# microsoft/StemGNN

Hardware: AMD Instinct MI355X
Metric: forecast-steps/sec (train) (higher is better)
Workload: dtype f32

## Files before the change

stemgnn_amd/csrc/gru.hip:

```cpp
#include <hip/hip_runtime.h>

#include "../../include/stemgnn_hip.h"
#include "gemm2.h"
#include "wgrad.h"
#include "dq_reduce.h"
#include "gemm_core.h"
#include "gru_wide.h"
#include "sg_host.h"

__device__ __forceinline__ float gru_sigmoid(float v) { return 1.f / (1.f + expf(-v)); }
__device__ __forceinline__ int gru_uniform(int v) { return __builtin_amdgcn_readfirstlane(v); }

struct GruGiOp {
  const float *x, *w_ih, *b_ih;
  float* gi;
  int B, S, Hd, W;
  unsigned *za, *zb;
  unsigned na, nb;
  __device__ bool setup(int, int& M, int& N, int& K0, int& K1) const {
    M = S * B; N = 3 * Hd; K0 = 0; K1 = W;
    if (na + nb) {
      const unsigned nwg = gridDim.x * gridDim.y, id = blockIdx.y * gridDim.x + blockIdx.x;
      const unsigned per = (na + nb + nwg - 1) / nwg, hi = min(na + nb, (id + 1) * per);
      for (unsigned i = id * per + threadIdx.x; i < hi; i += blockDim.x) {
// ... 201 lines not shown
    }
    __syncthreads();
    for (int item = wave; item < nwork; item += 16) {
      const int ub = item % nub, jq = item / nub;
      const int unit = ub * 64 + lane;
      const int uc = unit < Hd ? unit : Hd - 1;
      const int j0 = jq * jchunk, j1 = min(H3, j0 + jchunk);
      float a0 = 0.f;
      const float* wp = w_hh + (size_t)j0 * Hd + uc;
#pragma unroll 8
      for (int j = j0; j < j1; ++j) {
        a0 = fmaf(wp[0], dgh[j], a0);
        wp += Hd;
      }
      if (unit < Hd) part[jq * Hd + unit] = a0;
    }
    __syncthreads();
  }
}

typedef unsigned long long gru_u64;
__device__ __forceinline__ void gru_lds_barrier() {
#ifdef GRU_PLAIN_BARRIER
  __syncthreads();
#else
  asm volatile("s_waitcnt lgkmcnt(0)\n\ts_barrier" ::: "memory");
#endif
}
__device__ __forceinline__ void gru_publish(gru_u64* g, unsigned tag, float v) {
  __hip_atomic_store(g, ((gru_u64)tag << 32) | (gru_u64)__float_as_uint(v), __ATOMIC_RELAXED, __HIP_MEMORY_SCOPE_AGENT);
}
__device__ __forceinline__ float gru_consume(const gru_u64* g, unsigned tag, int* status) {
  gru_u64 x = __hip_atomic_load(g, __ATOMIC_RELAXED, __HIP_MEMORY_SCOPE_AGENT);
  unsigned spins = 0;
  while ((unsigned)(x >> 32) != tag) {
#ifndef GRU_NO_SLEEP
    __builtin_amdgcn_s_sleep(1);
#endif
    x = __hip_atomic_load(g, __ATOMIC_RELAXED, __HIP_MEMORY_SCOPE_AGENT);
    if (++spins > (1u << 22)) { atomicExch(status, 1); break; }
  }
  return __uint_as_float((unsigned)x);
}

__device__ __forceinline__ void gru_publish_x(gru_u64* g, unsigned tag, float v, bool same_xcd) {
  const gru_u64 x = ((gru_u64)tag << 32) | (gru_u64)__float_as_uint(v);
#if defined(GRU_PUB_PUSH) && GRU_PUB_PUSH == 3
  if (same_xcd) asm volatile("global_store_dwordx2 %0, %1, off sc0" : : "v"(g), "v"(x) : "memory");
#else
  if (same_xcd) asm volatile("global_store_dwordx2 %0, %1, off" : : "v"(g), "v"(x) : "memory");
#endif
  else __hip_atomic_store(g, x, __ATOMIC_RELAXED, __HIP_MEMORY_SCOPE_AGENT);
}
__device__ __forceinline__ bool gru_same_xcd(gru_u64* xid, int p, int P, int allow, int* status, int* s_flag, int tid) {
  if (tid == 0) {
    const unsigned xcc = __builtin_amdgcn_s_getreg(20 | (0 << 6) | (3 << 11)) & 0xfu;
    gru_publish(xid + p, 1u, (float)(xcc + 1));
    int same = allow;
    for (int q = 0; q < P; ++q) same &= gru_consume(xid + q, 1u, status) == (float)(xcc + 1);
    *s_flag = same;
  }
  __syncthreads();
  return *s_flag != 0;
}

struct GruCluster {
  int P, U, ncb, ksf, kcf, ksb, kcb;
};
__host__ __device__ inline GruCluster gru_cluster_geom(int Hd, int P) {
  GruCluster c;
  c.P = P;
  c.U = (Hd + P - 1) / P;
  c.ncb = (c.U + 63) / 64;
  c.ksf = 16 / (3 * c.ncb);
  c.kcf = c.ksf > 0 ? (Hd + c.ksf - 1) / c.ksf : 1 << 30;
  c.ksb = 16 / c.ncb;
  c.kcb = c.ksb > 0 ? (3 * Hd + c.ksb - 1) / c.ksb : 1 << 30;
  return c;
}
__device__ __forceinline__ void gru_cluster_ids(int B, int P, int& b, int& p) {
  const int id = blockIdx.x;
  const int bl = id & 7, r = id >> 3;
  p = r % P;
  b = (r / P) * 8 + bl;
  (void)B;
}

template <int KC, bool RS = true>
__global__ __launch_bounds__(1024) void gru_fwd_cluster_kernel(const float* __restrict__ gi, const float* __restrict__ w_hh,
                                                               const float* __restrict__ b_hh, int B, int S, int Hd, int P,
                                                               gru_u64* __restrict__ xbuf, int* __restrict__ status,
                                                               float* __restrict__ h_all, float* __restrict__ reserve) {
  extern __shared__ __attribute__((aligned(16))) float smem[];
  int b, p;
  gru_cluster_ids(B, P, b, p);
  if (b >= B) return;
  const GruCluster c = gru_cluster_geom(Hd, P);
  const int tid = threadIdx.x, lane = tid & 63, wave = tid >> 6;
  const int u0 = p * c.U;
  const int un = max(0, min(Hd, u0 + c.U) - u0);
  const int H3 = 3 * Hd;
  float* hs = smem;
  float* part = smem + Hd + KC;
  for (int i = tid; i < Hd + KC; i += 1024) hs[i] = 0.f;
  const int ncol = 3 * c.ncb;
  const bool has = wave < ncol * c.ksf;
  const int cb = has ? wave % ncol : 0, kq = has ? wave / ncol : 0;
  const int g = cb / c.ncb, ul = (cb % c.ncb) * 64 + lane;
  const int k0 = kq * c.kcf, kn = has ? max(0, min(Hd, k0 + c.kcf) - k0) : 0;
  float wr[KC];
  {
    const bool lane_ok = has && ul < un;
    const float* wrow = w_hh + ((size_t)g * Hd + (lane_ok ? u0 + ul : 0)) * Hd + (kn > 0 ? k0 : 0);
#pragma unroll
    for (int kk = 0; kk < KC; ++kk) {
      const float v = wrow[kk < kn ? kk : 0];
      wr[kk] = (lane_ok && kk < kn) ? v : 0.f;
    }
  }
  const int iu = tid < un ? tid : 0;
  const int gu = u0 + iu;
  const float bh0 = b_hh[gu], bh1 = b_hh[Hd + gu], bh2 = b_hh[2 * Hd + gu];
  __syncthreads();

  for (int s = 0; s < S; ++s) {
    const size_t row = (size_t)s * B + b;
    const float* gip = gi + row * H3;
    const float gp0 = gip[gu], gp1 = gip[Hd + gu], gp2 = gip[2 * Hd + gu];
    if (s > 0 && P > 1) {
      const gru_u64* xb = xbuf + ((size_t)(s & 1) * B + b) * Hd;
      for (int i = tid; i < Hd; i += 1024)
        if (i < u0 || i >= u0 + un) hs[i] = gru_consume(xb + i, (unsigned)s, status);
    }
    __syncthreads();
    if (has) {
      float a0 = 0.f, a1 = 0.f;
      const float* hk = hs + k0;
#pragma unroll
      for (int kk = 0; kk < KC; kk += 2) {
        if ((kk & 15) == 0) __builtin_amdgcn_sched_barrier(0);
        a0 = fmaf(wr[kk], hk[kk], a0);
        a1 = fmaf(wr[kk + 1], hk[kk + 1], a1);
      }
      if (ul < un) part[(kq * 3 + g) * c.U + ul] = a0 + a1;
    }
    __syncthreads();
    if (tid < un) {
      float g0 = bh0, g1 = bh1, g2 = bh2;
      for (int q = 0; q < c.ksf; ++q) {
        g0 += part[(q * 3 + 0) * c.U + iu];
        g1 += part[(q * 3 + 1) * c.U + iu];
        g2 += part[(q * 3 + 2) * c.U + iu];
      }
      const float r = gru_sigmoid(gp0 + g0);
      const float z = gru_sigmoid(gp1 + g1);
      const float n = tanhf(gp2 + r * g2);
      const float hn = (1.f - z) * n + z * hs[gu];
      if constexpr (RS) {
        float* rs = reserve + row * 4 * Hd;
        rs[gu] = r; rs[Hd + gu] = z; rs[2 * Hd + gu] = n; rs[3 * Hd + gu] = g2;
      }
      h_all[row * Hd + gu] = hn;
      hs[gu] = hn;
      if (P > 1 && s + 1 < S) gru_publish(xbuf + ((size_t)((s + 1) & 1) * B + b) * Hd + gu, (unsigned)(s + 1), hn);
    }
  }
}

template <int KC>
__global__ __launch_bounds__(1024) void gru_bwd_cluster_kernel(const float* __restrict__ dout, const float* __restrict__ w_hh,
                                                               const float* __restrict__ h_all, const float* __restrict__ reserve,
                                                               int B, int S, int Hd, int P, gru_u64* __restrict__ xbuf,
                                                               int* __restrict__ status, float* __restrict__ dgi,
                                                               float* __restrict__ dghn) {
  extern __shared__ __attribute__((aligned(16))) float smem[];
  int b, p;
  gru_cluster_ids(B, P, b, p);
  if (b >= B) return;
  const GruCluster c = gru_cluster_geom(Hd, P);
  const int tid = threadIdx.x, lane = tid & 63, wave = tid >> 6;
  const int u0 = p * c.U;
  const int un = max(0, min(Hd, u0 + c.U) - u0);
  const int H3 = 3 * Hd;
  float* dgh = smem;
  float* dhz = smem + H3 + KC;
  float* part = dhz + c.U;
  for (int i = tid; i < H3 + KC; i += 1024) dgh[i] = 0.f;
  for (int i = tid; i < c.U; i += 1024) dhz[i] = 0.f;
  for (int i = tid; i < c.ksb * c.U; i += 1024) part[i] = 0.f;
  const bool has = wave < c.ncb * c.ksb;
  const int cb = has ? wave % c.ncb : 0, jq = has ? wave / c.ncb : 0;
  const int ul = cb * 64 + lane;
  const int j0 = jq * c.kcb, jn = has ? max(0, min(H3, j0 + c.kcb) - j0) : 0;
  float wr[KC];
  {
    const bool lane_ok = has && ul < un;
    const float* wcol = w_hh + (size_t)(jn > 0 ? j0 : 0) * Hd + (lane_ok ? u0 + ul : 0);
#pragma unroll
    for (int jj = 0; jj < KC; ++jj) {
      const float v = wcol[(size_t)(jj < jn ? jj : 0) * Hd];
      wr[jj] = (lane_ok && jj < jn) ? v : 0.f;
    }
  }
  const int iu = tid < un ? tid : 0;
  const int gu = u0 + iu;
  __syncthreads();

  for (int s = S - 1; s >= 0; --s) {
    const size_t row = (size_t)s * B + b;
    const unsigned tag = (unsigned)(S - s);
    gru_u64* xb = xbuf + ((size_t)(tag & 1) * B + b) * H3;
    if (tid < un) {
      float dh = dout[row * Hd + gu] + dhz[iu];
      for (int q = 0; q < c.ksb; ++q) dh += part[q * c.U + iu];
      const float* rs = reserve + row * 4 * Hd;
      const float r = rs[gu], z = rs[Hd + gu], n = rs[2 * Hd + gu], ghn = rs[3 * Hd + gu];
      const float hp = h_all[(s > 0 ? row - B : row) * Hd + gu];
      const float hprev = s > 0 ? hp : 0.f;
      const float dn = dh * (1.f - z) * (1.f - n * n);
      const float dz = dh * (hprev - n) * z * (1.f - z);
      const float dr = dn * ghn * r * (1.f - r);
      const float dnr = dn * r;
      dgh[gu] = dr; dgh[Hd + gu] = dz; dgh[2 * Hd + gu] = dnr;
      dhz[iu] = dh * z;
      float* go = dgi + row * H3;
      go[gu] = dr; go[Hd + gu] = dz; go[2 * Hd + gu] = dn;
      dghn[row * Hd + gu] = dnr;
      if (P > 1 && s > 0) {
        gru_publish(xb + gu, tag, dr);
        gru_publish(xb + Hd + gu, tag, dz);
        gru_publish(xb + 2 * Hd + gu, tag, dnr);
      }
    }
    if (s == 0) break;
    if (P > 1) {
      for (int j = tid; j < H3; j += 1024) {
        const int k = j % Hd;
        if (k < u0 || k >= u0 + un) dgh[j] = gru_consume(xb + j, tag, status);
      }
    }
    __syncthreads();
    if (has) {
      float a0 = 0.f, a1 = 0.f;
      const float* gk = dgh + j0;
#pragma unroll
      for (int jj = 0; jj < KC; jj += 2) {
        if ((jj & 15) == 0) __builtin_amdgcn_sched_barrier(0);
        a0 = fmaf(wr[jj], gk[jj], a0);
        a1 = fmaf(wr[jj + 1], gk[jj + 1], a1);
      }
      if (ul < un) part[jq * c.U + ul] = a0 + a1;
    }
    __syncthreads();
  }
}

__device__ __forceinline__ float gru_bcast(float v, int src_lane) {
  return __builtin_bit_cast(float, __builtin_amdgcn_readlane(__builtin_bit_cast(int, v), src_lane));
}
typedef float gru_f2 __attribute__((ext_vector_type(2)));
#ifndef GRU_NR_FWD
#define GRU_NR_FWD 8
#endif
#ifndef GRU_NR_BWD
#define GRU_NR_BWD 16
#endif
#ifndef GRU_NR4
#define GRU_NR4 16
#endif
#define GRU_NR2(P, OW) (((OW) == 1 && (P) <= 4) ? GRU_NR_BWD : 64)
#define GRU_NR3(KU) ((KU) <= 58 ? GRU_NR_FWD : 32)
template <int KU, int NR>
struct GruBcast {
  static constexpr int NRK = NR < KU ? (NR & ~3) : ((KU + 3) & ~3);
  static constexpr int NL = NRK < KU ? (KU - NRK + 3) / 4 : 0;
  float4 v[NL > 0 ? NL : 1];
  float hv;
  __device__ __forceinline__ GruBcast(float hv_, float* lrow, int lane) : hv(hv_) {
    if constexpr (NL > 0) {
      lrow[lane] = hv_;
      asm volatile("" ::: "memory");
#pragma unroll
      for (int i = 0; i < NL; ++i) v[i] = *reinterpret_cast<const float4*>(lrow + NRK + 4 * i);
      __builtin_amdgcn_sched_barrier(0);
    }
  }
  __device__ __forceinline__ gru_f2 pair(int kk) const {
    if (kk < NRK) return gru_f2{gru_bcast(hv, kk), gru_bcast(hv, kk + 1)};
    const float4 t = v[NL > 0 ? (kk - NRK) >> 2 : 0];
    return ((kk - NRK) & 2) ? gru_f2{t.z, t.w} : gru_f2{t.x, t.y};
  }
};
template <int KU, int NR>
__device__ __forceinline__ float gru_matvec(const gru_f2 (&wr)[32], float hv, float* lrow, int lane) {
  const GruBcast<KU, NR> bc(hv, lrow, lane);
  gru_f2 a0 = {0.f, 0.f}, a1 = {0.f, 0.f};
#pragma unroll
  for (int kk = 0; kk + 3 < KU; kk += 4) {
    a0 = __builtin_elementwise_fma(wr[kk >> 1], bc.pair(kk), a0);
    a1 = __builtin_elementwise_fma(wr[(kk >> 1) + 1], bc.pair(kk + 2), a1);
  }
  if constexpr ((KU & 3) != 0) a0 = __builtin_elementwise_fma(wr[(KU - 2) >> 1], bc.pair(KU - 2), a0);
  return (a0.x + a1.x) + (a0.y + a1.y);
}
__device__ __forceinline__ float gru_poll_lane(const gru_u64* g, unsigned tag, bool active, int* status) {
  float v = 0.f;
  if (active) v = gru_consume(g, tag, status);
  return v;
}

#ifdef GRU_PROF
#define GRU_T(var) const long long var = (long long)__builtin_readcyclecounter()
#define GRU_ACC(acc, t1, t0) acc += (t1) - (t0)
#else
#define GRU_T(var)
#define GRU_ACC(acc, t1, t0)
#endif
template <int KU, int NR>
__device__ __forceinline__ void gru_matvec3(const gru_f2 (&w0)[32], const gru_f2 (&w1)[32], const gru_f2 (&w2)[32],
                                            float hv, float* lrow, int lane, float& o0, float& o1, float& o2) {
  const GruBcast<KU, NR> bc(hv, lrow, lane);
  gru_f2 a0 = {0.f, 0.f}, b0 = {0.f, 0.f}, a1 = {0.f, 0.f}, b1 = {0.f, 0.f}, a2 = {0.f, 0.f}, b2 = {0.f, 0.f};
#pragma unroll
  for (int kk = 0; kk + 3 < KU; kk += 4) {
    const gru_f2 h0 = bc.pair(kk), h1 = bc.pair(kk + 2);
    a0 = __builtin_elementwise_fma(w0[kk >> 1], h0, a0);
    a1 = __builtin_elementwise_fma(w1[kk >> 1], h0, a1);
    a2 = __builtin_elementwise_fma(w2[kk >> 1], h0, a2);
    b0 = __builtin_elementwise_fma(w0[(kk >> 1) + 1], h1, b0);
    b1 = __builtin_elementwise_fma(w1[(kk >> 1) + 1], h1, b1);
    b2 = __builtin_elementwise_fma(w2[(kk >> 1) + 1], h1, b2);
  }
  if constexpr ((KU & 3) != 0) {
    const gru_f2 h0 = bc.pair(KU - 2);
    a0 = __builtin_elementwise_fma(w0[(KU - 2) >> 1], h0, a0);
    a1 = __builtin_elementwise_fma(w1[(KU - 2) >> 1], h0, a1);
    a2 = __builtin_elementwise_fma(w2[(KU - 2) >> 1], h0, a2);
  }
  o0 = (a0.x + b0.x) + (a0.y + b0.y);
  o1 = (a1.x + b1.x) + (a1.y + b1.y);
  o2 = (a2.x + b2.x) + (a2.y + b2.y);
}
constexpr int GRU_PACK_KMAX = 40;
template <int KU, int NR>
__device__ __forceinline__ void gru_matvec2(const gru_f2 (&w0)[GRU_PACK_KMAX / 2], const gru_f2 (&w1)[GRU_PACK_KMAX / 2],
                                            float hv, float* lrow, int lane, float& o0, float& o1) {
  static_assert(KU <= GRU_PACK_KMAX && (KU & 1) == 0, "packed mat-vec: slices of at most 40 units");
  const GruBcast<KU, NR> bc(hv, lrow, lane);
  gru_f2 a0 = {0.f, 0.f}, b0 = {0.f, 0.f}, a1 = {0.f, 0.f}, b1 = {0.f, 0.f};
#pragma unroll
  for (int kk = 0; kk + 3 < KU; kk += 4) {
    const gru_f2 h0 = bc.pair(kk), h1 = bc.pair(kk + 2);
    a0 = __builtin_elementwise_fma(w0[kk >> 1], h0, a0);
    a1 = __builtin_elementwise_fma(w1[kk >> 1], h0, a1);
    b0 = __builtin_elementwise_fma(w0[(kk >> 1) + 1], h1, b0);
    b1 = __builtin_elementwise_fma(w1[(kk >> 1) + 1], h1, b1);
  }
  if constexpr ((KU & 3) != 0) {
    const gru_f2 h0 = bc.pair(KU - 2);
    a0 = __builtin_elementwise_fma(w0[(KU - 2) >> 1], h0, a0);
    a1 = __builtin_elementwise_fma(w1[(KU - 2) >> 1], h0, a1);
  }
  o0 = (a0.x + b0.x) + (a0.y + b0.y);
  o1 = (a1.x + b1.x) + (a1.y + b1.y);
}
template <int P, int KU, int OW>
__global__ __launch_bounds__(3 * (P / OW) * 64) void gru_bwd_cluster2_kernel(const float* __restrict__ dout, const float* __restrict__ w_hh,
                                                                      const float* __restrict__ h_all,
                                                                      const float* __restrict__ reserve, int B, int S, int Hd,
                                                                      gru_u64* __restrict__ xbuf, int* __restrict__ status,
                                                                      float* __restrict__ dgi, float* __restrict__ dghn,
                                                                      int s_hi, int s_lo, float* __restrict__ carry,
                                                                      int s_mark, unsigned* __restrict__ progress,
                                                                      gru_u64* __restrict__ xid, int allow_fast) {
  static_assert(P % OW == 0, "owners per wave");
  constexpr int NTH = 3 * (P / OW) * 64;
  __shared__ float part[2][3 * P][64];
  __shared__ __attribute__((aligned(16))) float lrow[3 * P][64];
  __shared__ int s_fast;
  int b, p;
  gru_cluster_ids(B, P, b, p);
  if (b >= B) return;
  const bool fast = P > 1 && gru_same_xcd(xid + (size_t)b * P, p, P, allow_fast, status, &s_fast, threadIdx.x);
  const int U = (Hd + P - 1) / P;
  const int tid = threadIdx.x, lane = tid & 63;
  const int wave = gru_uniform(tid >> 6);
  const int g = wave / (P / OW), q0 = (wave - g * (P / OW)) * OW;
  const int u0 = p * U, un = max(0, min(Hd, u0 + U) - u0);
  const int H3 = 3 * Hd;
  gru_f2 wr[OW][32];
  int k0[OW], kn[OW];
#pragma unroll
  for (int o = 0; o < OW; ++o) {
    k0[o] = ((q0 + o + p) % P) * U;
    kn[o] = max(0, min(Hd, k0[o] + U) - k0[o]);
    const bool lane_ok = lane < un;
    const float* wcol = w_hh + ((size_t)g * Hd + (kn[o] > 0 ? k0[o] : 0)) * Hd + (lane_ok ? u0 + lane : 0);
#pragma unroll
    for (int kk = 0; kk < KU; ++kk) {
      const float v = wcol[(size_t)(kk < kn[o] ? kk : 0) * Hd];
      wr[o][kk >> 1][kk & 1] = (lane_ok && kk < kn[o]) ? v : 0.f;
    }
  }
  const int gu = u0 + (tid < un ? tid : 0);
  float dhz = s_hi < S - 1 ? carry[(size_t)b * Hd + gu] : 0.f;
  for (int i = tid; i < 2 * 3 * P * 64; i += NTH) (&part[0][0][0])[i] = 0.f;
  size_t prow = (size_t)s_hi * B + b;
  float p_do = dout[prow * Hd + gu];
  float p_r = reserve[prow * 4 * Hd + gu], p_z = reserve[prow * 4 * Hd + Hd + gu];
  float p_n = reserve[prow * 4 * Hd + 2 * Hd + gu], p_g = reserve[prow * 4 * Hd + 3 * Hd + gu];
  float p_h = h_all[(s_hi > 0 ? prow - B : prow) * Hd + gu];
  __syncthreads();

#ifdef GRU_PROF
  long long c_poll = 0, c_mv = 0, c_bar = 0, c_gate = 0;
#endif
  for (int s = s_hi; s >= s_lo; --s) {
    const size_t row = (size_t)s * B + b;
    const unsigned tag = (unsigned)(S - s);
    gru_u64* xb = xbuf + ((size_t)(tag & 1) * B + b) * H3;
    float own_dr = 0.f;
    GRU_T(t0);
    if (tid < un) {
      float dh = p_do + dhz;
#pragma unroll
      for (int w = 0; w < 3 * P; ++w) dh += part[(tag + 1) & 1][w][tid];
      const float r = p_r, z = p_z, n = p_n, ghn = p_g;
      const float hprev = s > 0 ? p_h : 0.f;
      const float dn = dh * (1.f - z) * (1.f - n * n);
      const float dz = dh * (hprev - n) * z * (1.f - z);
      const float dr = dn * ghn * r * (1.f - r);
      const float dnr = dn * r;
      own_dr = dr;
      dhz = dh * z;
      if (s > 0) {
        gru_publish_x(xb + gu, tag, dr, fast);
        gru_publish_x(xb + Hd + gu, tag, dz, fast);
        gru_publish_x(xb + 2 * Hd + gu, tag, dnr, fast);
        const size_t rn = row - B;
        p_do = dout[rn * Hd + gu];
        p_r = reserve[rn * 4 * Hd + gu]; p_z = reserve[rn * 4 * Hd + Hd + gu];
        p_n = reserve[rn * 4 * Hd + 2 * Hd + gu]; p_g = reserve[rn * 4 * Hd + 3 * Hd + gu];
        p_h = h_all[(s > 1 ? rn - B : rn) * Hd + gu];
      }
      float* go = dgi + row * H3;
      go[gu] = dr; go[Hd + gu] = dz; go[2 * Hd + gu] = dn;
      dghn[row * Hd + gu] = dnr;
    }
    if (s == 0) break;
    GRU_T(t1);
    GRU_ACC(c_gate, t1, t0);
#pragma unroll
    for (int o = 0; o < OW; ++o) {
      float dv;
      if (wave == 0 && o == 0) dv = own_dr;
      else dv = gru_poll_lane(xb + (size_t)g * Hd + k0[o] + (lane < kn[o] ? lane : 0), tag, lane < kn[o], status);
#ifdef GRU_PROF
      GRU_T(t2);
      GRU_ACC(c_poll, t2, t1);
#endif
      part[tag & 1][g * P + q0 + o][lane] = gru_matvec<KU, GRU_NR2(P, OW)>(wr[o], dv, lrow[wave * OW + o], lane);
#ifdef GRU_PROF
      GRU_T(t3);
      GRU_ACC(c_mv, t3, t2);
#endif
    }
    GRU_T(t4);
    gru_lds_barrier();
    GRU_T(t5);
    GRU_ACC(c_bar, t5, t4);
    if (s == s_mark) {
      asm volatile("s_waitcnt vmcnt(0)" ::: "memory");
      __syncthreads();
      if (tid == 0) {
        __builtin_amdgcn_fence(__ATOMIC_RELEASE, "agent");
        asm volatile("s_waitcnt vmcnt(0)" ::: "memory");
        __hip_atomic_fetch_add(progress, 1u, __ATOMIC_RELAXED, __HIP_MEMORY_SCOPE_AGENT);
      }
    }
  }
#ifdef GRU_PROF
  if (blockIdx.x == 0 && lane == 0)
    printf("gru bwd2 wave %d: per step cycles: gate phase %lld  poll/own %lld  matvec %lld  barrier wait %lld  (S=%d)\n", wave,
           c_gate / S, c_poll / S, c_mv / S, c_bar / S, S);
#endif
  if (s_lo > 0 && tid < un) {
    const unsigned tag = (unsigned)(S - s_lo);
    float c = dhz;
#pragma unroll
    for (int w = 0; w < 3 * P; ++w) c += part[tag & 1][w][tid];
    carry[(size_t)b * Hd + gu] = c;
  }
}

#include "gru_cluster4.h"

struct GruWhhGradOp {
  const float *dgi, *dghn, *h_all;
  float* part;
  int B, S, Hd, nsplit, chunk;
  __device__ bool setup(int z, int& M, int& N, int& K0, int& K1) const {
    M = 3 * Hd; N = Hd + 1; K0 = z * chunk; K1 = min(S * B, K0 + chunk);
    return true;
  }
  __device__ float a(int, int i, int k) const {
    const float* p = i < 2 * Hd ? dgi + (size_t)k * 3 * Hd + i : dghn + (size_t)k * Hd + (i - 2 * Hd);
    return *p;
  }
  __device__ float b(int, int k, int j) const {
    const float v = h_all[(size_t)(k >= B ? k - B : 0) * Hd + (j < Hd ? j : Hd - 1)];
    return j >= Hd ? 1.f : (k >= B ? v : 0.f);
  }
  __device__ void epi(int z, int i, int j, float v) const { part[((size_t)z * 3 * Hd + i) * (Hd + 1) + j] = v; }
};
struct GruWihGradOp {
  const float *dgi, *x;
  float* part;
  int B, S, Hd, W, nsplit, chunk;
  int row0, rows;
  __device__ bool setup(int z, int& M, int& N, int& K0, int& K1) const {
    M = 3 * Hd; N = W + 1; K0 = row0 + z * chunk; K1 = min(row0 + rows, K0 + chunk);
    return true;
  }
  __device__ float a(int, int i, int k) const { return dgi[(size_t)k * 3 * Hd + i]; }
  __device__ float b(int, int k, int j) const {
    const int s = k / B, bb = k - s * B;
    const float v = x[((size_t)bb * W + (j < W ? j : W - 1)) * S + s];
    return j < W ? v : 1.f;
  }
  __device__ void epi(int z, int i, int j, float v) const { part[((size_t)z * 3 * Hd + i) * (W + 1) + j] = v; }
};

struct GruReduceJobs {
  const float* part[3];
  float* out_w[3];
  float* out_b[3];
  int rows[3], cols[3], nsplit[3];
};
__global__ void gru_reduce_grad_kernel(const GruReduceJobs J) {
  const int job = blockIdx.y;
  const int nsplit = J.nsplit[job];
  const int rows = J.rows[job], cols = J.cols[job];
  const size_t idx = (size_t)blockIdx.x * blockDim.x + threadIdx.x;
  const size_t slab = (size_t)rows * (cols + 1);
  if (idx >= slab) return;
  const float* part = J.part[job];
  float s = 0.f;
  for (int z = 0; z < nsplit; z += 8) {
    float v[8];
#pragma unroll
    for (int u = 0; u < 8; ++u) {
      const int zz = z + u;
      const float x = part[(size_t)(zz < nsplit ? zz : 0) * slab + idx];
      v[u] = zz < nsplit ? x : 0.f;
    }
#pragma unroll
    for (int u = 0; u < 8; ++u) s += v[u];
  }
  const int j = (int)(idx / (cols + 1)), k = (int)(idx - (size_t)j * (cols + 1));
  if (k < cols) J.out_w[job][(size_t)j * cols + k] = s;
  else J.out_b[job][j] = s;
}

#include <stdlib.h>
static int gru_nsplit() { return 32; }
#define GRU_NSPLIT gru_nsplit()
static int gru_ih_slabs(int B) { return B > gru_nsplit() ? B : gru_nsplit(); }

extern "C" size_t stemgnn_gru_reserve_floats(int B, int S, int Hd) { return (size_t)4 * S * B * Hd; }
#define GRU_KC 48
static int gru_limit_of_cus(int cus) { return cus - cus / 8; }
static int gru_resident_limit() {
  static int cached_dev = -1, cached = 0;
  int dev = 0;
  if (hipGetDevice(&dev) != hipSuccess) return 0;
  if (dev != cached_dev) {
    int cus = 0;
    if (hipDeviceGetAttribute(&cus, hipDeviceAttributeMultiprocessorCount, dev) != hipSuccess) return 0;
    cached = gru_limit_of_cus(cus);
    cached_dev = dev;
  }
  return cached;
}
static int gru_pick_P(int B, int Hd, int limit) {
  const char* e = getenv("STEMGNN_GRU_CLUSTER");
  if (e && atoi(e) == 0) return 0;
  for (int P = 1; P <= 8; P *= 2) {
    const GruCluster c = gru_cluster_geom(Hd, P);
    if (c.ksf >= 1 && c.ksb >= 1 && c.kcf <= GRU_KC && c.kcb <= GRU_KC && B * P <= limit) return P;
  }
  return 0;
}
static int gru_pick_P2(int B, int Hd, int limit) {
  const char* e = getenv("STEMGNN_GRU_CLUSTER");
  if (e && atoi(e) != 2) return 0;
  static const int cand[6] = {1, 2, 4, 5, 6, 8};
  for (int i = 0; i < 6; ++i) {
    const int P = cand[i];
    if ((Hd + P - 1) / P <= 64 && B * P <= limit) return P;
  }
  return 0;
}
template <int P>
static size_t gru_lds_hog(const void* fn) {
  const size_t bytes = (size_t)156 * 1024 - sizeof(float) * 3 * 3 * P * 64;
  (void)hipFuncSetAttribute(fn, hipFuncAttributeMaxDynamicSharedMemorySize, (int)bytes);
// ... 561 lines not shown
```

stemgnn_amd/csrc/gru_cluster4.h:

```cpp
#pragma once

#ifndef GRU_PUB_PUSH
#define GRU_PUB_PUSH 0
#endif
__device__ __forceinline__ void gru4_after_publish(const gru_u64* g) {
#if GRU_PUB_PUSH == 1
  asm volatile("s_waitcnt vmcnt(0)" ::: "memory");
#elif GRU_PUB_PUSH == 2
  gru_u64 x;
  asm volatile("global_load_dwordx2 %0, %1, off sc1" : "=v"(x) : "v"(g) : "memory");
  asm volatile("" :: "v"(x));
#else
  (void)g;
#endif
}
#ifndef GRU_POLL_MODE
#define GRU_POLL_MODE 0
#endif
#ifndef GRU_POLL_PRE_F
#define GRU_POLL_PRE_F 9
#endif
#ifndef GRU_POLL_PRE_B
#define GRU_POLL_PRE_B 9
#endif
#ifndef GRU_POLL_LOOP_SLEEP
#define GRU_POLL_LOOP_SLEEP 1
#endif
#include "gru_math.h"

template <int PRE>
__device__ __forceinline__ float gru4_poll(const gru_u64* g, unsigned tag, bool active, int* status) {
  if (PRE > 0) __builtin_amdgcn_s_sleep(PRE);
#if (GRU_POLL_MODE & 1)
  float v = 0.f;
  if (active) {
    gru_u64 a = __hip_atomic_load(g, __ATOMIC_RELAXED, __HIP_MEMORY_SCOPE_AGENT);
    __builtin_amdgcn_s_sleep(2);
    gru_u64 b = __hip_atomic_load(g, __ATOMIC_RELAXED, __HIP_MEMORY_SCOPE_AGENT);
    unsigned spins = 0;
    for (;;) {
      if ((unsigned)(a >> 32) == tag) { v = __uint_as_float((unsigned)a); break; }
      a = __hip_atomic_load(g, __ATOMIC_RELAXED, __HIP_MEMORY_SCOPE_AGENT);
      if ((unsigned)(b >> 32) == tag) { v = __uint_as_float((unsigned)b); break; }
      b = __hip_atomic_load(g, __ATOMIC_RELAXED, __HIP_MEMORY_SCOPE_AGENT);
      if (++spins > (1u << 22)) { atomicExch(status, 1); break; }
    }
  }
  return v;
#else
  float v = 0.f;
  if (active) {
    gru_u64 x = __hip_atomic_load(g, __ATOMIC_RELAXED, __HIP_MEMORY_SCOPE_AGENT);
    unsigned spins = 0;
    while ((unsigned)(x >> 32) != tag) {
      if (GRU_POLL_LOOP_SLEEP > 0) __builtin_amdgcn_s_sleep(GRU_POLL_LOOP_SLEEP);
      x = __hip_atomic_load(g, __ATOMIC_RELAXED, __HIP_MEMORY_SCOPE_AGENT);
      if (++spins > (1u << 22)) { atomicExch(status, 1); break; }
    }
    v = __uint_as_float((unsigned)x);
  }
  return v;
#endif
}
template <int PRE>
__device__ __forceinline__ void gru4_poll2(const gru_u64* g0, const gru_u64* g1, unsigned tag, bool act0, bool act1,
                                           int* status, float (&v)[2]) {
  if (PRE > 0) __builtin_amdgcn_s_sleep(PRE);
  gru_u64 x0 = __hip_atomic_load(g0, __ATOMIC_RELAXED, __HIP_MEMORY_SCOPE_AGENT);
  gru_u64 x1 = __hip_atomic_load(g1, __ATOMIC_RELAXED, __HIP_MEMORY_SCOPE_AGENT);
  unsigned spins = 0;
  while (act0 && (unsigned)(x0 >> 32) != tag) {
    if (GRU_POLL_LOOP_SLEEP > 0) __builtin_amdgcn_s_sleep(GRU_POLL_LOOP_SLEEP);
    x0 = __hip_atomic_load(g0, __ATOMIC_RELAXED, __HIP_MEMORY_SCOPE_AGENT);
    if (++spins > (1u << 22)) { atomicExch(status, 1); break; }
  }
  spins = 0;
  while (act1 && (unsigned)(x1 >> 32) != tag) {
    if (GRU_POLL_LOOP_SLEEP > 0) __builtin_amdgcn_s_sleep(GRU_POLL_LOOP_SLEEP);
    x1 = __hip_atomic_load(g1, __ATOMIC_RELAXED, __HIP_MEMORY_SCOPE_AGENT);
    if (++spins > (1u << 22)) { atomicExch(status, 1); break; }
  }
  v[0] = act0 ? __uint_as_float((unsigned)x0) : 0.f;
  v[1] = act1 ? __uint_as_float((unsigned)x1) : 0.f;
}
#ifndef GRU_FWD_PACK
#define GRU_FWD_PACK 1
#endif
#ifndef GRU_PART_VEC
#define GRU_PART_VEC 1
#endif
constexpr int gru4_part_stride(int n) { return 4 * (((n + 3) / 4) | 1); }
template <int ROWS, int N, int P = 0>
struct Gru4Part {
  static constexpr int PS = gru4_part_stride(N);
  static constexpr int FLOATS = GRU_PART_VEC ? ROWS * PS : ROWS * N;
  static __device__ __forceinline__ int at(int row, int q) {
#if GRU_PART_VEC
    return row * PS + q;
#else
    return P > 0 ? ((row >> 6) * P + q) * 64 + (row & 63) : q * ROWS + row;
#endif
  }
  static __device__ __forceinline__ float sum(const float* part, int row, float acc) {
#if GRU_PART_VEC
    float4 v[PS / 4];
#pragma unroll
    for (int i = 0; i < (N + 3) / 4; ++i) v[i] = *reinterpret_cast<const float4*>(part + row * PS + 4 * i);
#pragma unroll
    for (int q = 0; q < N; ++q) {
      const float4 t = v[q >> 2];
      acc += (q & 3) == 0 ? t.x : ((q & 3) == 1 ? t.y : ((q & 3) == 2 ? t.z : t.w));
    }
#else
#pragma unroll
    for (int q = 0; q < N; ++q) acc += part[at(row, q)];
#endif
    return acc;
  }
};
constexpr int gru4_static_lds_floats(int P, int nin, int nout) {
  return 2 * 64 * (GRU_PART_VEC ? gru4_part_stride(3 * P) : 3 * P) + 3 * P * 64 + 2 * nin * 64 + 2 * nout * 64;
}

constexpr bool gru4_fwd_packs(int KU) { return GRU_FWD_PACK != 0 && KU > 32 && KU <= 40; }
constexpr size_t gru4_fwd_hog_bytes(int P, int KU) {
  return gru4_fwd_packs(KU)
             ? (size_t)156 * 1024 - sizeof(float) * (2 * 128 * (GRU_PART_VEC ? gru4_part_stride(P) : P) + P * 64 + 2 * 3 * 64 + 2 * 5 * 64)
             : 0;
}
constexpr int GRU4_WMAX = 16;
#ifndef GRU_CHORE_SLEEP_F
#define GRU_CHORE_SLEEP_F 16
#endif
#ifndef GRU_SW_MODE
#define GRU_SW_MODE 0
#endif
#ifndef GRU_SW_SLEEP
#define GRU_SW_SLEEP 30
#endif
#ifndef GRU_CHORE_SLEEP_B
#define GRU_CHORE_SLEEP_B 10
#endif
template <int P, int KU, bool RS = true>
__global__ __launch_bounds__((P + 2) * 64) void gru_fwd_cluster4_kernel(const float* __restrict__ gi, const float* __restrict__ w_hh,
                                                                        const float* __restrict__ b_hh, int B, int S, int Hd,
                                                                        gru_u64* __restrict__ xbuf, int* __restrict__ status,
                                                                        float* __restrict__ h_all, float* __restrict__ reserve,
                                                                        gru_u64* __restrict__ xid, int allow_fast) {
  constexpr bool PACK = gru4_fwd_packs(KU);
  typedef Gru4Part<PACK ? 128 : 192, P, PACK ? 0 : P> Part;
  __shared__ __attribute__((aligned(16))) float part[2][Part::FLOATS];
  __shared__ __attribute__((aligned(16))) float lrow[P][64];
  __shared__ float gin[2][3][64];
  __shared__ float stash[2][5][64];
  __shared__ int s_fast;
  int b, p;
  gru_cluster_ids(B, P, b, p);
  if (b >= B) return;
  const bool fast = P > 1 && gru_same_xcd(xid + (size_t)b * P, p, P, allow_fast, status, &s_fast, threadIdx.x);
  const int U = (Hd + P - 1) / P;
  const int tid = threadIdx.x, lane = tid & 63;
  const int wave = gru_uniform(tid >> 6);
  const int u0 = p * U, un = max(0, min(Hd, u0 + U) - u0);
  const int H3 = 3 * Hd;
  const bool lane_ok = lane < un;
  const int gu = u0 + (lane_ok ? lane : 0);
  if (un == 0) return;

  if (wave < P) {
    const int q = wave;
    const int k0 = ((q + p) % P) * U, kn = max(0, min(Hd, k0 + U) - k0);
    gru_f2 wr[3][32];
    gru_f2 wp[2][GRU_PACK_KMAX / 2];
    if constexpr (PACK) {
#pragma unroll
      for (int t = 0; t < 2; ++t) {
        const int o = 64 * t + lane, g = o / U, u = o - g * U;
        const bool live = o < 3 * U && u < un;
        const float* wrow = w_hh + (live ? ((size_t)g * Hd + u0 + u) * Hd : (size_t)0) + (kn > 0 ? k0 : 0);
#pragma unroll
        for (int kk = 0; kk < KU; ++kk) {
          const float v = wrow[kk < kn ? kk : 0];
          wp[t][kk >> 1][kk & 1] = (live && kk < kn) ? v : 0.f;
        }
      }
    } else {
#pragma unroll
      for (int g = 0; g < 3; ++g) {
        const float* wrow = w_hh + ((size_t)g * Hd + gu) * Hd + (kn > 0 ? k0 : 0);
#pragma unroll
        for (int kk = 0; kk < KU; ++kk) {
          const float v = wrow[kk < kn ? kk : 0];
          wr[g][kk >> 1][kk & 1] = (lane_ok && kk < kn) ? v : 0.f;
        }
      }
    }
    const gru_u64* pollp = xbuf + (size_t)b * Hd + k0 + (lane < kn ? lane : 0);
    const size_t par = (size_t)B * Hd;
#ifdef GRU_PROF
    long long c_a = 0, c_b = 0, c_c = 0;
#endif
    for (int s = 0; s < S; ++s) {
      GRU_T(t0);
      float hv = 0.f;
      if (s > 0) hv = gru4_poll<GRU_POLL_PRE_F>(pollp + (s & 1) * par, (unsigned)s, lane < kn, status);
      GRU_T(t1);
      GRU_ACC(c_a, t1, t0);
      float* pw = part[s & 1];
      if constexpr (PACK) {
        float o0, o1;
        gru_matvec2<KU, GRU_NR3(KU)>(wp[0], wp[1], hv, lrow[q], lane, o0, o1);
        pw[Part::at(lane, q)] = o0;
        pw[Part::at(64 + lane, q)] = o1;
      } else {
        float o0, o1, o2;
        gru_matvec3<KU, GRU_NR3(KU)>(wr[0], wr[1], wr[2], hv, lrow[q], lane, o0, o1, o2);
        pw[Part::at(lane, q)] = o0;
        pw[Part::at(64 + lane, q)] = o1;
        pw[Part::at(128 + lane, q)] = o2;
      }
      GRU_T(t2);
      GRU_ACC(c_b, t2, t1);
      gru_lds_barrier();
      GRU_T(t3);
      GRU_ACC(c_c, t3, t2);
    }
    gru_lds_barrier();
#ifdef GRU_PROF
    if (blockIdx.x == 0 && lane == 0)
      printf("gru fwd4 mat-vec wave %d: per step cycles: poll %lld  matvec %lld  barrier wait %lld\n", wave, c_a / S, c_b / S, c_c / S);
#endif
  } else if (wave == P + 1) {
    const float* gip = gi + (size_t)b * H3 + gu;
    const size_t grow = (size_t)B * H3;
    float v0 = gip[0], v1 = gip[Hd], v2 = gip[2 * Hd];
    for (int s = 0; s < S; ++s) {
      gin[s & 1][0][lane] = v0;
      gin[s & 1][1][lane] = v1;
      gin[s & 1][2][lane] = v2;
      float r = 0.f, z = 0.f, n = 0.f, g2 = 0.f, hn = 0.f;
      if (s >= 2) {
        r = stash[s & 1][0][lane]; z = stash[s & 1][1][lane]; n = stash[s & 1][2][lane];
        g2 = stash[s & 1][3][lane]; hn = stash[s & 1][4][lane];
      }
      if (s > 0) __builtin_amdgcn_s_sleep(GRU_CHORE_SLEEP_F);
      if (s + 1 < S) {
        const float* gn = gip + (size_t)(s + 1) * grow;
        v0 = gn[0]; v1 = gn[Hd]; v2 = gn[2 * Hd];
      }
      if (s >= 2 && lane_ok) {
        const size_t rw = (size_t)(s - 2) * B + b;
        if constexpr (RS) {
          float* rs = reserve + rw * 4 * Hd + gu;
          rs[0] = r; rs[Hd] = z; rs[2 * Hd] = n; rs[3 * Hd] = g2;
        }
        h_all[rw * Hd + gu] = hn;
      }
      gru_lds_barrier();
    }
    gru_lds_barrier();
    for (int t = (S >= 2 ? S - 2 : S - 1); t < S; ++t) {
      const size_t rw = (size_t)t * B + b;
      if (lane_ok) {
        if constexpr (RS) {
          float* rs = reserve + rw * 4 * Hd + gu;
          rs[0] = stash[t & 1][0][lane]; rs[Hd] = stash[t & 1][1][lane]; rs[2 * Hd] = stash[t & 1][2][lane];
          rs[3 * Hd] = stash[t & 1][3][lane];
        }
        h_all[rw * Hd + gu] = stash[t & 1][4][lane];
      }
    }
  } else {
    const float bh0 = b_hh[gu], bh1 = b_hh[Hd + gu], bh2 = b_hh[2 * Hd + gu];
    float hown = 0.f;
    const int row0 = PACK ? (lane < U ? lane : 0) : lane, rstep = PACK ? U : 64;
    gru_u64* pub = xbuf + (size_t)b * Hd + gu;
    const size_t par = (size_t)B * Hd;
#ifdef GRU_PROF
    long long c_a = 0, c_b = 0, c_c = 0;
#endif
    for (int s = 0; s < S; ++s) {
      GRU_T(t0);
      gru_lds_barrier();
      GRU_T(t1);
      GRU_ACC(c_a, t1, t0);
      const float* pr = part[s & 1];
      const float g0 = Part::sum(pr, row0, bh0), g1 = Part::sum(pr, row0 + rstep, bh1), g2 = Part::sum(pr, row0 + 2 * rstep, bh2);
      const float gp0 = gin[s & 1][0][lane], gp1 = gin[s & 1][1][lane], gp2 = gin[s & 1][2][lane];
      const float r = gru4_sigmoid(gp0 + g0);
      const float z = gru4_sigmoid(gp1 + g1);
      const float n = gru4_tanh(gp2 + r * g2);
      const float hn = (1.f - z) * n + z * hown;
      hown = hn;
      if (s + 1 < S && lane_ok) gru_publish_x(pub + ((s + 1) & 1) * par, (unsigned)(s + 1), hn, fast);
      gru4_after_publish(pub);
      GRU_T(t2);
      GRU_ACC(c_b, t2, t1);
      stash[s & 1][0][lane] = r;
      stash[s & 1][1][lane] = z;
      stash[s & 1][2][lane] = n;
      stash[s & 1][3][lane] = g2;
      stash[s & 1][4][lane] = hn;
      GRU_T(t3);
      GRU_ACC(c_c, t3, t2);
    }
    gru_lds_barrier();
#ifdef GRU_PROF
    if (blockIdx.x == 0 && lane == 0)
      printf("gru fwd4 gate wave: per step cycles: barrier wait %lld  gate phase to publish %lld  stash %lld\n", c_a / S, c_b / S, c_c / S);
#endif
  }
}

template <int P, int KU, int OW = 1, bool SW = false>
__global__ __launch_bounds__((3 * P / OW + 2 + (SW ? 1 : 0)) * 64) void gru_bwd_cluster4_kernel(const float* __restrict__ dout, const float* __restrict__ w_hh,
                                                                            const float* __restrict__ h_all,
                                                                            const float* __restrict__ reserve, int B, int S, int Hd,
                                                                            gru_u64* __restrict__ xbuf, int* __restrict__ status,
                                                                            float* __restrict__ dgi, float* __restrict__ dghn,
                                                                            gru_u64* __restrict__ xid, int allow_fast,
                                                                            const float* __restrict__ x, float* __restrict__ ih_slab,
                                                                            int W, const float* __restrict__ dkey,
                                                                            const float* __restrict__ dquery,
                                                                            const float* __restrict__ wk, const float* __restrict__ wq,
                                                                            unsigned* __restrict__ prog, int prog_ts) {
  static_assert(P % OW == 0 && (OW == 1 || OW == 2), "owner slices per wave");
  constexpr int NMV = 3 * P / OW;
  typedef Gru4Part<64, NMV> Part;
  __shared__ __attribute__((aligned(16))) float part[2][Part::FLOATS];
  __shared__ __attribute__((aligned(16))) float lrow[NMV][64];
  __shared__ float bin[2][6][64];
  __shared__ float bout[2][4][64];
  __shared__ int s_fast;
  int b, p;
  gru_cluster_ids(B, P, b, p);
  if (b >= B) return;
  const bool fast = P > 1 && gru_same_xcd(xid + (size_t)b * P, p, P, allow_fast, status, &s_fast, threadIdx.x);
  const int U = (Hd + P - 1) / P;
  const int tid = threadIdx.x, lane = tid & 63;
  const int wave = gru_uniform(tid >> 6);
  const int u0 = p * U, un = max(0, min(Hd, u0 + U) - u0);
  const int H3 = 3 * Hd;
  const bool lane_ok = lane < un;
  const int gu = u0 + (lane_ok ? lane : 0);
  for (int i = tid; i < 2 * Part::FLOATS; i += (int)blockDim.x) (&part[0][0])[i] = 0.f;

  if (wave < NMV) {
    const int g = wave / (P / OW), q0 = (wave - g * (P / OW)) * OW;
    gru_f2 wr[OW][32];
    int kn[OW];
    const gru_u64* pollp[OW];
#pragma unroll
    for (int o = 0; o < OW; ++o) {
      const int k0 = ((q0 + o + p) % P) * U;
      kn[o] = max(0, min(Hd, k0 + U) - k0);
      const float* wcol = w_hh + ((size_t)g * Hd + (kn[o] > 0 ? k0 : 0)) * Hd + gu;
#pragma unroll
      for (int kk = 0; kk < KU; ++kk) {
        const float v = wcol[(size_t)(kk < kn[o] ? kk : 0) * Hd];
        wr[o][kk >> 1][kk & 1] = (lane_ok && kk < kn[o]) ? v : 0.f;
      }
      pollp[o] = xbuf + (size_t)b * H3 + (size_t)g * Hd + k0 + (lane < kn[o] ? lane : 0);
    }
    const size_t par = (size_t)B * H3;
#ifdef GRU_PROF
    long long c_a = 0, c_b = 0, c_c = 0;
#endif
    gru_lds_barrier();
    for (int s = S - 1; s >= 1; --s) {
      const unsigned tag = (unsigned)(S - s);
      GRU_T(t0);
      float pv;
      if constexpr (OW == 1) {
        const float dv = gru4_poll<GRU_POLL_PRE_B>(pollp[0] + (tag & 1) * par, tag, lane < kn[0], status);
        pv = gru_matvec<KU, (KU <= 58 ? GRU_NR4 : (GRU_NR4 > 24 ? GRU_NR4 : 24))>(wr[0], dv, lrow[wave], lane);
      } else {
        float dv[2];
        gru4_poll2<GRU_POLL_PRE_B>(pollp[0] + (tag & 1) * par, pollp[1] + (tag & 1) * par, tag, lane < kn[0], lane < kn[1],
                                   status, dv);
        pv = gru_matvec<KU, 64>(wr[0], dv[0], lrow[wave], lane);
        pv += gru_matvec<KU, 64>(wr[OW - 1], dv[1], lrow[wave], lane);
      }
      part[tag & 1][Part::at(lane, wave)] = pv;
      GRU_T(t2);
      GRU_ACC(c_b, t2, t0);
      gru_lds_barrier();
      GRU_T(t3);
      GRU_ACC(c_c, t3, t2);
    }
    gru_lds_barrier();
#ifdef GRU_PROF
    if (blockIdx.x == 0 && lane == 0)
      printf("gru bwd4 mat-vec wave %d: per step cycles: poll %lld  matvec %lld  barrier wait %lld\n", wave, c_a / S, c_b / S, c_c / S);
#endif
  } else if (wave == NMV + 1) {
    const bool factored = dkey != nullptr;
    const float dk_own = factored ? dkey[(size_t)b * Hd + gu] : 0.f, dq_own = factored ? dquery[(size_t)b * Hd + gu] : 0.f;
    auto fetch = [&](int t, float (&val)[6]) {
      const size_t rw = (size_t)t * B + b;
      const float* rs = reserve + rw * 4 * Hd + gu;
      val[0] = factored ? dk_own * wk[t] + dq_own * wq[t] : dout[rw * Hd + gu];
      val[1] = rs[0]; val[2] = rs[Hd]; val[3] = rs[2 * Hd]; val[4] = rs[3 * Hd];
      val[5] = t > 0 ? h_all[(rw - B) * Hd + gu] : 0.f;
    };
    auto stage = [&](int t, const float (&val)[6]) {
#pragma unroll
      for (int v = 0; v < 6; ++v) bin[t & 1][v][lane] = val[v];
    };
    constexpr bool wt = SW;
    auto put = [&](size_t rw, float dr, float dz, float dn, float dnr) {
      if (wt) return;
      float* go = dgi + rw * H3 + gu;
      go[0] = dr; go[Hd] = dz; go[2 * Hd] = dn;
      dghn[rw * Hd + gu] = dnr;
    };
    auto flush = [&](int t) {
      const size_t rw = (size_t)t * B + b;
      const float dr = bout[t & 1][0][lane], dz = bout[t & 1][1][lane], dn = bout[t & 1][2][lane], dnr = bout[t & 1][3][lane];
      if (lane_ok) put(rw, dr, dz, dn, dnr);
    };
    float acc[3][GRU4_WMAX], accb[3] = {0.f, 0.f, 0.f};
#pragma unroll
    for (int g = 0; g < 3; ++g)
#pragma unroll
      for (int w = 0; w < GRU4_WMAX; ++w) acc[g][w] = 0.f;
    const float* xrow = x + (size_t)b * W * S;
    auto wih_x = [&](int t, float (&xv)[GRU4_WMAX]) {
      if (!ih_slab) return;
#pragma unroll
      for (int w = 0; w < GRU4_WMAX; ++w) xv[w] = xrow[(size_t)(w < W ? w : 0) * S + t];
    };
    auto wih = [&](const float (&xv)[GRU4_WMAX], float dr, float dz, float dn) {
      if (!ih_slab) return;
      accb[0] += dr; accb[1] += dz; accb[2] += dn;
#pragma unroll
      for (int w = 0; w < GRU4_WMAX; ++w) {
        acc[0][w] = fmaf(dr, xv[w], acc[0][w]);
        acc[1][w] = fmaf(dz, xv[w], acc[1][w]);
        acc[2][w] = fmaf(dn, xv[w], acc[2][w]);
      }
    };
    float val[6];
    fetch(S - 1, val);
    stage(S - 1, val);
    if (S >= 2) fetch(S - 2, val);
    gru_lds_barrier();
    for (int s = S - 1; s >= 1; --s) {
      stage(s - 1, val);
      float dr = 0.f, dz = 0.f, dn = 0.f, dnr = 0.f;
      const bool have = s + 1 <= S - 1;
      if (have) { dr = bout[(s + 1) & 1][0][lane]; dz = bout[(s + 1) & 1][1][lane]; dn = bout[(s + 1) & 1][2][lane]; dnr = bout[(s + 1) & 1][3][lane]; }
      float xv[GRU4_WMAX];
      if (have) wih_x(s + 1, xv);
      __builtin_amdgcn_s_sleep(GRU_CHORE_SLEEP_B);
      if (s >= 2) fetch(s - 2, val);
      if (have && lane_ok) put((size_t)(s + 1) * B + b, dr, dz, dn, dnr);
      if (have) wih(xv, dr, dz, dn);
      gru_lds_barrier();
    }
    gru_lds_barrier();
    float xv[GRU4_WMAX];
    if (S >= 2) { flush(1); wih_x(1, xv); wih(xv, bout[1][0][lane], bout[1][1][lane], bout[1][2][lane]); }
    flush(0);
    wih_x(0, xv);
    wih(xv, bout[0][0][lane], bout[0][1][lane], bout[0][2][lane]);
    if (ih_slab && lane_ok) {
#pragma unroll
      for (int g = 0; g < 3; ++g) {
        float* o = ih_slab + ((size_t)b * H3 + (size_t)g * Hd + gu) * (W + 1);
#pragma unroll
        for (int w = 0; w < GRU4_WMAX; ++w)
          if (w < W) o[w] = acc[g][w];
        o[W] = accb[g];
      }
    }
  } else if (SW && wave == NMV + 2) {
    auto put = [&](int t) {
      const size_t rw = (size_t)t * B + b;
      const float dr = bout[t & 1][0][lane], dz = bout[t & 1][1][lane], dn = bout[t & 1][2][lane], dnr = bout[t & 1][3][lane];
      if (lane_ok) {
        float* go = dgi + rw * H3 + gu;
#if GRU_SW_MODE == 0
        __hip_atomic_store(go, dr, __ATOMIC_RELAXED, __HIP_MEMORY_SCOPE_AGENT);
        __hip_atomic_store(go + Hd, dz, __ATOMIC_RELAXED, __HIP_MEMORY_SCOPE_AGENT);
        __hip_atomic_store(go + 2 * Hd, dn, __ATOMIC_RELAXED, __HIP_MEMORY_SCOPE_AGENT);
        __hip_atomic_store(dghn + rw * Hd + gu, dnr, __ATOMIC_RELAXED, __HIP_MEMORY_SCOPE_AGENT);
#elif GRU_SW_MODE == 2
        go[0] = dr; go[Hd] = dz; go[2 * Hd] = dn; dghn[rw * Hd + gu] = dnr;
#elif GRU_SW_MODE == 3
        __builtin_nontemporal_store(dr, go); __builtin_nontemporal_store(dz, go + Hd);
        __builtin_nontemporal_store(dn, go + 2 * Hd); __builtin_nontemporal_store(dnr, dghn + rw * Hd + gu);
#else
        if (dr + dz + dn + dnr == 1.2345e-30f) go[0] = dr;
#endif
      }
    };
    auto count = [&](int t) {
      if (lane == 0) __hip_atomic_fetch_add(prog + t / prog_ts, 1u, __ATOMIC_RELAXED, __HIP_MEMORY_SCOPE_AGENT);
    };
    gru_lds_barrier();
    for (int s = S - 1; s >= 1; --s) {
      __builtin_amdgcn_s_sleep(GRU_SW_SLEEP);
      if (s + 1 <= S - 1) put(s + 1);
      if (s + 3 <= S - 1 && (s + 3) % prog_ts == 0) {
        asm volatile("s_waitcnt vmcnt(8)" ::: "memory");
        count(s + 3);
      }
      gru_lds_barrier();
    }
    gru_lds_barrier();
    if (S >= 2) put(1);
    put(0);
    asm volatile("s_waitcnt vmcnt(0)" ::: "memory");
    for (int t = (S - 1 < 3 ? S - 1 : 3); t >= 0; --t)
      if (t % prog_ts == 0) count(t);
  } else {
    float dhz = 0.f;
    gru_u64* pub = xbuf + (size_t)b * H3 + gu;
    const size_t par = (size_t)B * H3;
#ifdef GRU_PROF
    long long c_a = 0, c_b = 0, c_c = 0;
#endif
    gru_lds_barrier();
    for (int s = S - 1; s >= 0; --s) {
      const unsigned tag = (unsigned)(S - s);
      GRU_T(t1);
      const float dh = Part::sum(part[(tag + 1) & 1], lane, bin[s & 1][0][lane] + dhz);
      const float r = bin[s & 1][1][lane], z = bin[s & 1][2][lane], n = bin[s & 1][3][lane], ghn = bin[s & 1][4][lane];
      const float hprev = s > 0 ? bin[s & 1][5][lane] : 0.f;
      const float dn = dh * (1.f - z) * (1.f - n * n);
      const float dz = dh * (hprev - n) * z * (1.f - z);
      const float dr = dn * ghn * r * (1.f - r);
      const float dnr = dn * r;
      dhz = dh * z;
      if (s > 0 && lane_ok) {
        gru_u64* xb = pub + (tag & 1) * par;
        gru_publish_x(xb, tag, dr, fast);
        gru_publish_x(xb + Hd, tag, dz, fast);
        gru_publish_x(xb + 2 * Hd, tag, dnr, fast);
      }
      gru4_after_publish(pub);
      GRU_T(t2);
      GRU_ACC(c_b, t2, t1);
      bout[s & 1][0][lane] = dr;
      bout[s & 1][1][lane] = dz;
      bout[s & 1][2][lane] = dn;
      bout[s & 1][3][lane] = dnr;
      GRU_T(t3);
      GRU_ACC(c_c, t3, t2);
      if (s > 0) gru_lds_barrier();
      GRU_T(t4);
      GRU_ACC(c_a, t4, t3);
    }
    gru_lds_barrier();
#ifdef GRU_PROF
    if (blockIdx.x == 0 && lane == 0)
      printf("gru bwd4 gate wave: per step cycles: barrier wait %lld  gate phase to publish %lld  stash %lld\n", c_a / S, c_b / S, c_c / S);
#endif
  }
}
```

Measured before the change: 88320.

## Fold backward GRU mat-vec across wave halves with permlane32 swap reduction

In the backward cluster kernel's mat-vec waves (when OW is 1 and KU exceeds 32), each lane now owns two output units and half of the K range. The broadcast vector is read from LDS as float pairs, and the two half-wave partial sums are combined with permlane32_swap. This replaces the per-lane full-K readlane/broadcast mat-vec and should shorten the serial per-step latency on the recurrence critical path. The output row mapping is permuted to match the new ownership, and the chore-wave sleep is lowered for the folded path, which shifts how the waves are balanced.

```diff
diff --git a/stemgnn_amd/csrc/gru.hip b/stemgnn_amd/csrc/gru.hip
--- a/stemgnn_amd/csrc/gru.hip
+++ b/stemgnn_amd/csrc/gru.hip
@@ -527,6 +527,31 @@
   }
   if constexpr ((KU & 3) != 0) a0 = __builtin_elementwise_fma(wr[(KU - 2) >> 1], bc.pair(KU - 2), a0);
   return (a0.x + a1.x) + (a0.y + a1.y);
+}
+constexpr int gru_fold_pairs(int KU) { return (KU + 3) / 4; }
+constexpr int GRU_FOLD_PMAX = 16;
+template <int KU>
+__device__ __forceinline__ float gru_matvec_fold(const gru_f2 (&w)[2][GRU_FOLD_PMAX], float dv, float* lrow, int lane) {
+  static_assert(KU <= 64 && (KU & 1) == 0, "folded mat-vec: slices of at most 64 units");
+  constexpr int NP = gru_fold_pairs(KU);
+  lrow[lane] = dv;
+  asm volatile("" ::: "memory");
+  const float* lr = lrow + ((lane >> 5) << 1);
+  gru_f2 d[NP];
+#pragma unroll
+  for (int i = 0; i < NP; ++i) d[i] = *reinterpret_cast<const gru_f2*>(lr + 4 * i);
+  __builtin_amdgcn_sched_barrier(0);
+  gru_f2 c0 = {0.f, 0.f}, c1 = {0.f, 0.f};
+#pragma unroll
+  for (int i = 0; i < NP; ++i) {
+    c0 = __builtin_elementwise_fma(w[0][i], d[i], c0);
+    c1 = __builtin_elementwise_fma(w[1][i], d[i], c1);
+  }
+  auto swap_add = [](float a, float b) {
+    const auto r = __builtin_amdgcn_permlane32_swap(__builtin_bit_cast(unsigned, a), __builtin_bit_cast(unsigned, b), false, false);
+    return __builtin_bit_cast(float, (unsigned)r[0]) + __builtin_bit_cast(float, (unsigned)r[1]);
+  };
+  return swap_add(swap_add(c0.x, c0.y), swap_add(c1.x, c1.y));
 }
 __device__ __forceinline__ float gru_poll_lane(const gru_u64* g, unsigned tag, bool active, int* status) {
   float v = 0.f;
diff --git a/stemgnn_amd/csrc/gru_cluster4.h b/stemgnn_amd/csrc/gru_cluster4.h
--- a/stemgnn_amd/csrc/gru_cluster4.h
+++ b/stemgnn_amd/csrc/gru_cluster4.h
@@ -86,6 +86,9 @@
 #ifndef GRU_FWD_PACK
 #define GRU_FWD_PACK 1
 #endif
+#ifndef GRU_BWD_FOLD
+#define GRU_BWD_FOLD 1
+#endif
 #ifndef GRU_PART_VEC
 #define GRU_PART_VEC 1
 #endif
@@ -123,6 +126,7 @@
 }
 
 constexpr bool gru4_fwd_packs(int KU) { return GRU_FWD_PACK != 0 && KU > 32 && KU <= 40; }
+constexpr bool gru4_bwd_folds(int KU, int OW) { return GRU_BWD_FOLD != 0 && OW == 1 && KU > 32; }
 constexpr size_t gru4_fwd_hog_bytes(int P, int KU) {
   return gru4_fwd_packs(KU)
              ? (size_t)156 * 1024 - sizeof(float) * (2 * 128 * (GRU_PART_VEC ? gru4_part_stride(P) : P) + P * 64 + 2 * 3 * 64 + 2 * 5 * 64)
@@ -139,7 +143,10 @@
 #define GRU_SW_SLEEP 30
 #endif
 #ifndef GRU_CHORE_SLEEP_B
-#define GRU_CHORE_SLEEP_B 10
+#define GRU_CHORE_SLEEP_B 7
+#endif
+#ifndef GRU_CHORE_SLEEP_B_RL
+#define GRU_CHORE_SLEEP_B_RL 10
 #endif
 template <int P, int KU, bool RS = true>
 __global__ __launch_bounds__((P + 2) * 64) void gru_fwd_cluster4_kernel(const float* __restrict__ gi, const float* __restrict__ w_hh,
@@ -326,6 +333,7 @@
                                                                             unsigned* __restrict__ prog, int prog_ts) {
   static_assert(P % OW == 0 && (OW == 1 || OW == 2), "owner slices per wave");
   constexpr int NMV = 3 * P / OW;
+  constexpr bool FOLD = gru4_bwd_folds(KU, OW);
   typedef Gru4Part<64, NMV> Part;
   __shared__ __attribute__((aligned(16))) float part[2][Part::FLOATS];
   __shared__ __attribute__((aligned(16))) float lrow[NMV][64];
@@ -348,20 +356,40 @@
   if (wave < NMV) {
     const int g = wave / (P / OW), q0 = (wave - g * (P / OW)) * OW;
     gru_f2 wr[OW][32];
+    gru_f2 wf[2][GRU_FOLD_PMAX];
     int kn[OW];
     const gru_u64* pollp[OW];
 #pragma unroll
     for (int o = 0; o < OW; ++o) {
       const int k0 = ((q0 + o + p) % P) * U;
       kn[o] = max(0, min(Hd, k0 + U) - k0);
-      const float* wcol = w_hh + ((size_t)g * Hd + (kn[o] > 0 ? k0 : 0)) * Hd + gu;
-#pragma unroll
-      for (int kk = 0; kk < KU; ++kk) {
-        const float v = wcol[(size_t)(kk < kn[o] ? kk : 0) * Hd];
-        wr[o][kk >> 1][kk & 1] = (lane_ok && kk < kn[o]) ? v : 0.f;
+      if constexpr (FOLD) {
+        const int half = lane >> 5;
+#pragma unroll
+        for (int t = 0; t < 2; ++t) {
+          const int j = 2 * (lane & 31) + t;
+          const bool live = j < un;
+          const float* wcol = w_hh + ((size_t)g * Hd + (kn[o] > 0 ? k0 : 0)) * Hd + u0 + (live ? j : 0);
+#pragma unroll
+          for (int i = 0; i < gru_fold_pairs(KU); ++i)
+#pragma unroll
+            for (int c = 0; c < 2; ++c) {
+              const int kk = 4 * i + 2 * half + c;
+              const float v = wcol[(size_t)(kk < kn[o] ? kk : 0) * Hd];
+              wf[t][i][c] = (live && kk < kn[o]) ? v : (kk < KU ? 0.f : -0.f);
+            }
+        }
+      } else {
+        const float* wcol = w_hh + ((size_t)g * Hd + (kn[o] > 0 ? k0 : 0)) * Hd + gu;
+#pragma unroll
+        for (int kk = 0; kk < KU; ++kk) {
+          const float v = wcol[(size_t)(kk < kn[o] ? kk : 0) * Hd];
+          wr[o][kk >> 1][kk & 1] = (lane_ok && kk < kn[o]) ? v : 0.f;
+        }
       }
       pollp[o] = xbuf + (size_t)b * H3 + (size_t)g * Hd + k0 + (lane < kn[o] ? lane : 0);
     }
+    const int prow = FOLD ? 2 * (lane & 31) + (lane >> 5) : lane;
     const size_t par = (size_t)B * H3;
 #ifdef GRU_PROF
     long long c_a = 0, c_b = 0, c_c = 0;
@@ -373,7 +401,8 @@
       float pv;
       if constexpr (OW == 1) {
         const float dv = gru4_poll<GRU_POLL_PRE_B>(pollp[0] + (tag & 1) * par, tag, lane < kn[0], status);
-        pv = gru_matvec<KU, (KU <= 58 ? GRU_NR4 : (GRU_NR4 > 24 ? GRU_NR4 : 24))>(wr[0], dv, lrow[wave], lane);
+        if constexpr (FOLD) pv = gru_matvec_fold<KU>(wf, dv, lrow[wave], lane);
+        else pv = gru_matvec<KU, (KU <= 58 ? GRU_NR4 : (GRU_NR4 > 24 ? GRU_NR4 : 24))>(wr[0], dv, lrow[wave], lane);
       } else {
         float dv[2];
         gru4_poll2<GRU_POLL_PRE_B>(pollp[0] + (tag & 1) * par, pollp[1] + (tag & 1) * par, tag, lane < kn[0], lane < kn[1],
@@ -381,7 +410,7 @@
         pv = gru_matvec<KU, 64>(wr[0], dv[0], lrow[wave], lane);
         pv += gru_matvec<KU, 64>(wr[OW - 1], dv[1], lrow[wave], lane);
       }
-      part[tag & 1][Part::at(lane, wave)] = pv;
+      part[tag & 1][Part::at(prow, wave)] = pv;
       GRU_T(t2);
       GRU_ACC(c_b, t2, t0);
       gru_lds_barrier();
@@ -452,7 +481,7 @@
       if (have) { dr = bout[(s + 1) & 1][0][lane]; dz = bout[(s + 1) & 1][1][lane]; dn = bout[(s + 1) & 1][2][lane]; dnr = bout[(s + 1) & 1][3][lane]; }
       float xv[GRU4_WMAX];
       if (have) wih_x(s + 1, xv);
-      __builtin_amdgcn_s_sleep(GRU_CHORE_SLEEP_B);
+      __builtin_amdgcn_s_sleep(FOLD ? GRU_CHORE_SLEEP_B : GRU_CHORE_SLEEP_B_RL);
       if (s >= 2) fetch(s - 2, val);
       if (have && lane_ok) put((size_t)(s + 1) * B + b, dr, dz, dn, dnr);
       if (have) wih(xv, dr, dz, dn);
```

After: 90560, median of 6. +2.5%, better.
